# Cyruscxy/TinyPathTracer

Hardware: AMD Instinct MI355X
Metric: Mrays/s at 1920x1080x1024spp (box.gltf, 8 bounces); achieved GB/s vs peak (higher is better)
Workload: dtype f32

## Files before the change

### tinypathtracer_amd/csrc/common/device_api.hpp

```cpp
#pragma once

#include <hip/hip_runtime_api.h>
#include <stdint.h>

namespace tpt {

struct DevLight {
    int32_t type;
    float color[3];
    float intensity;
    float pos[3];
    float dir[3];
    float cos_outer;
    float inv_cos_cone_diff;
};

constexpr int kMaxLights = 16;
constexpr int kRngJumps = 16;
constexpr int kJumpWords = 160 * 5;

struct TraceArgs {
    const float4* inner;
    const float4* inner4;
    int32_t n4;
    int32_t lds_nodes;
    int32_t lds_nodes_offset;
    const float4* tri;
    const float4* shade;
    const float4* mtl;
    int32_t n_faces;
    int32_t n_materials;
    int32_t n_lights;
    int32_t stack_depth;
    const DevLight* lights;
    const uint32_t* env;
    int32_t env_w, env_h;
    int32_t is_b, is_bw, is_bh;
    const float* is_cond;
    const float* is_row;
    const float* is_marg;
    float is_total;
    const int32_t* is_guide_r;
    const int32_t* is_guide_c;
    int32_t is_kr, is_kc;
    int32_t env_is;
    float c2w[16];
    float origin[3];
    float sensor_w, sensor_h;
    float half_sw, half_sh;
    float inv_w, inv_h;
    int32_t width, height;
    int32_t band_rows, band_count, band_index, band_height;
    const int32_t* band_list;
    unsigned long long* band_cost;
    int32_t n_frames;
    int32_t max_depth;
    int32_t samples;
    int32_t flags;
    int32_t refill;
    int32_t leaf_kb;
    int32_t boxes_finite;
    int32_t any_emitter;
    int32_t emit_root;
    float4 emit_box[8];
    int32_t n_emit_box;
    const float4* sliver_groups;
    const float4* sliver_list;
    int32_t n_sliver_groups;
    float cull_eps;
    int32_t graze;
    int32_t pair;
    int32_t drained;
    int32_t quad;
    int32_t xcd_run;
    int32_t xcd_rot;
    int32_t lds_rec_offset;
    int32_t rec_lds_levels;
    int32_t stack_lds_slots;
    int32_t lds_stack_offset;
    int32_t lds_mtl_offset;
    int32_t mtl_in_lds;
    uint32_t* rng;
    float* accum;
    unsigned long long* counters;
    unsigned long long* debug_waves;
};

struct ResolveArgs {
    const float* accum;
    float* radiance;
    uint8_t* bgra;
    int32_t width, height;
    int32_t band_rows, band_count, band_index, band_height;
    const int32_t* band_list;
    int32_t spp;
};

hipError_t launch_rng_init(const uint32_t* jumps, uint64_t seed, int32_t width, int32_t band_rows,
                           int32_t band_count, int32_t band_index, const int32_t* band_list, int32_t band_height,
                           int32_t height, uint32_t* rng, hipStream_t s);
hipError_t launch_rng_init_linear(const uint32_t* jumps, uint64_t seed, uint64_t first, uint32_t n,
                                  uint32_t* states_aos, hipStream_t s);

struct BuildBuffers {
    int32_t n_faces, n_vertices, n_objects, n_materials;
    const uint32_t* indices;
    const float* vertices;
    const float* normals;
    const int2* lut;
    const float* vert_trans;
    const float* normal_trans;
    const float4* mtl;
    float* wverts;
    float* wnorms;
    unsigned long long* keys;
    unsigned long long* keys_sorted;
// ... 193 lines not shown
```

### tinypathtracer_amd/csrc/common/trace_variant.hpp

```cpp
#pragma once

#include <algorithm>
#include <cstddef>
#include <cstdint>
#include <type_traits>

#ifndef TPT_TRACE_WAVES
#define TPT_TRACE_WAVES 5
#endif
#ifndef TPT_TRACE_WAVES_IS
#define TPT_TRACE_WAVES_IS 4
#endif
#ifndef TPT_TRACE_WAVES_PAIR
#define TPT_TRACE_WAVES_PAIR 4
#endif
#ifndef TPT_TRACE_WAVES_DRAIN
#define TPT_TRACE_WAVES_DRAIN 4
#endif
#ifndef TPT_TRACE_WAVES_QUAD
#define TPT_TRACE_WAVES_QUAD 4
#endif

#ifdef TPT_WG_WAVES
#define TPT_WGW(n) TPT_WG_WAVES
#else
#define TPT_WGW(n) n
#endif
#define TPT_WGW_LANE TPT_WGW(1)
#define TPT_WGW_DRAIN TPT_WGW(1)
#define TPT_WGW_PAIR TPT_WGW(4)
#define TPT_WGW_IS TPT_WGW(4)
#define TPT_WGW_QUAD TPT_WGW(4)
#define TPT_WGW_REF TPT_WGW(4)
#ifndef TPT_MTL_LDS_MAX
#define TPT_MTL_LDS_MAX 2048
#endif

namespace tpt {

enum TraceFamily : int { TF_LANE, TF_DRAIN, TF_PAIR, TF_IS, TF_QUAD, TF_REF, TF_IS_PAIR, TF_REF_IS, kTraceFamilies };
constexpr int kTracePublicFamilies = 6;

struct TraceFamilyInfo {
    int wgw;
    int waves;
    int lds_waves;
    int lanes;
    int tile_w, tile_rows;
    bool env_is, ordered;
};
inline constexpr TraceFamilyInfo kTraceFamily[kTraceFamilies] = {
     {TPT_WGW_LANE, TPT_TRACE_WAVES, TPT_TRACE_WAVES, 1, 16, 16, false, true},
     {TPT_WGW_DRAIN, TPT_TRACE_WAVES_DRAIN, TPT_TRACE_WAVES, 1, 16, 16, false, true},
     {TPT_WGW_PAIR, TPT_TRACE_WAVES_PAIR, TPT_TRACE_WAVES_PAIR, 2, 16, 8, false, true},
     {TPT_WGW_IS, TPT_TRACE_WAVES_IS, TPT_TRACE_WAVES_IS, 1, 16, 16, true, true},
     {TPT_WGW_QUAD, TPT_TRACE_WAVES_QUAD, TPT_TRACE_WAVES_QUAD, 4, 8, 8, false, true},
     {TPT_WGW_REF, TPT_TRACE_WAVES, TPT_TRACE_WAVES, 1, 16, 16, false, false},
     {TPT_WGW_IS, TPT_TRACE_WAVES_IS, TPT_TRACE_WAVES_IS, 2, 16, 8, true, true},
     {TPT_WGW_REF, TPT_TRACE_WAVES_IS, TPT_TRACE_WAVES, 1, 16, 16, true, false},
};

struct TraceKey {
    TraceFamily family;
    bool deep;
    bool lights;
    bool mtl_lds;
    bool wide_ids;
    bool noemit;
};
constexpr int kTraceKeyBits = 8;
constexpr unsigned trace_key_pack(const TraceKey& k) {
    return (unsigned)k.family | k.deep << 3 | k.lights << 4 | k.mtl_lds << 5 | k.wide_ids << 6 | k.noemit << 7;
}
constexpr TraceKey trace_key_unpack(unsigned p) {
    return {(TraceFamily)(p & 7), (p >> 3 & 1) != 0, (p >> 4 & 1) != 0, (p >> 5 & 1) != 0, (p >> 6 & 1) != 0, (p >> 7 & 1) != 0};
}
constexpr bool trace_key_legal(const TraceKey& k) {
    const TraceFamilyInfo& f = kTraceFamily[k.family];
    if (!f.ordered && !(k.deep && k.lights && !k.mtl_lds && k.wide_ids)) return false;
    if (k.lights ? f.lanes == 4 : (f.lanes == 2 || f.env_is)) return false;
    return !k.noemit || f.lanes == 2;
}

template <TraceFamily F, int MAXD_, bool LIGHTS_, bool MTL_LDS_, typename StackT_, bool NOEMIT_>
struct TraceVariant {
    static_assert((MAXD_ == 8 || MAXD_ == 64) && (std::is_same_v<StackT_, uint16_t> || std::is_same_v<StackT_, int>));
    static constexpr TraceKey key{F, MAXD_ == 64, LIGHTS_, MTL_LDS_, sizeof(StackT_) == 4, NOEMIT_};
    static_assert(trace_key_legal(key), "no such k_trace variant (trace_key_legal)");
    static constexpr TraceFamilyInfo fam = kTraceFamily[F];
    static_assert(fam.wgw == 1 || fam.wgw == 2 || fam.wgw == 4, "waves per k_trace workgroup: 1, 2 or 4");
    static constexpr int MAXD = MAXD_, WGW = fam.wgw, WAVES = fam.waves;
    static constexpr bool ORDERED = fam.ordered, LIGHTS = LIGHTS_, MTL_LDS = MTL_LDS_, ENVIS = fam.env_is,
                          PAIR = fam.lanes == 2, DRAIN = F == TF_DRAIN, QUAD = fam.lanes == 4, NOEMIT = NOEMIT_;
    using StackT = StackT_;
};

constexpr uint32_t kNoProbe = 0x7fffu;
constexpr int rec_words(int n_lights, int n_materials) {
    return (n_lights > 0 || n_materials + 1 >= (int)kNoProbe) ? 5 : 2;
}
constexpr bool trace_small_ids(int n_faces) { return 2 * (size_t)n_faces - 1 <= 65535; }
constexpr bool trace_mtl_in_lds(int n_materials) { return (size_t)(n_materials + 1) * 32 <= (size_t)TPT_MTL_LDS_MAX; }
constexpr bool trace_five_words(bool ref_order, bool env_is, int n_lights, int n_materials) {
    return ref_order || env_is || rec_words(n_lights, n_materials) == 5;
}

struct TraceSelectIn {
    bool ref_order, env_is, pair, quad, drained;
    int n_lights, n_materials, n_faces, max_depth;
    bool any_emitter;
};
struct TraceSelection {
    TraceKey key;
    const char* error;
};
constexpr TraceSelection select_trace_variant(const TraceSelectIn& in) {
    if (in.ref_order) return {{in.env_is ? TF_REF_IS : TF_REF, true, true, false, true, false}, nullptr};
    const bool pair = in.pair && (in.env_is || in.n_lights > 0) && in.n_materials + 1 < (int)kNoProbe;
    TraceKey k{TF_LANE, in.max_depth > 8, trace_five_words(false, in.env_is, in.n_lights, in.n_materials),
               trace_mtl_in_lds(in.n_materials), !trace_small_ids(in.n_faces), pair && !in.any_emitter};
    if (in.env_is) k.family = pair ? TF_IS_PAIR : TF_IS;
    else if (in.quad) k.family = TF_QUAD;
    else if (pair) k.family = TF_PAIR;
    else if (in.drained) k.family = TF_DRAIN;
    return {k, trace_key_legal(k) ? nullptr : "four lanes per pixel need 2-word path records"};
}

struct TraceLds {
    size_t bytes;
    int mtl_offset, stack_offset, rec_offset;
    int stack_slots, rec_levels;
};
constexpr size_t kLdsSlack = 512;

inline TraceLds trace_lds_layout(const TraceKey& k, int wgw, int stack_depth, int max_depth, int n_materials,
                                 size_t max_slots = (size_t)-1, size_t max_levels = (size_t)-1) {
    const TraceFamilyInfo& f = kTraceFamily[k.family];
    size_t lds_budget = ((163840 / (size_t)f.lds_waves) & ~(size_t)255) * (size_t)wgw / 4;
    if (wgw < 4) lds_budget -= kLdsSlack * (size_t)wgw;
    const size_t row = 64 * (size_t)wgw;
    const size_t mtl_bytes = k.mtl_lds ? ((size_t)(n_materials + 1) * 2 * 16 + 127) / 128 * 128 : 0;
    const size_t budget = lds_budget - mtl_bytes;
    const size_t elem = k.wide_ids ? 4 : 2;
    const size_t slot = f.lanes == 4 ? row / 4 * elem : row * elem;
    const size_t level = (size_t)(k.lights ? 5 : 2) * (f.lanes == 2 ? row / 2 : row) * sizeof(float);
    size_t slots = std::min((size_t)stack_depth + 3, max_slots);
    const size_t want = std::min(std::min<size_t>((size_t)max_depth, (budget - 12 * slot) / level), max_levels);
    if (slots * slot + want * level > budget)
// ... 9 lines not shown
```

### tinypathtracer_amd/csrc/host/api_internal.hpp

```cpp
#pragma once

#include <hip/hip_runtime_api.h>

#include <algorithm>
#include <cstring>
#include <memory>
#include <string>
#include <thread>
#include <vector>

#include "../common/device_api.hpp"
#include "../common/ptrig.hpp"
#include "../common/tpt_math.hpp"
#include "launch_plan.hpp"
#include "tpt.h"
#include "tpt_internal.hpp"

namespace tpt {
namespace host __attribute__((visibility("hidden"))) {

tpt_status fail(tpt_status st, const std::string& msg);

#define HIP_OR_FAIL(expr)                                                                             \
    do {                                                                                              \
// ... 178 lines not shown
    int n4 = -1, need = 0, ne4 = -1, eneed = 0;
    tpt_status st = TPT_OK;
    std::string msg;
    tpt::WideWorkspace ws;
    std::thread th;
    ~HostTrees() { join(); }
    void join() {
        if (th.joinable()) th.join();
    }
    void reset_results() {
        n4 = -1;
        need = 0;
        ne4 = -1;
        eneed = 0;
        st = TPT_OK;
        msg.clear();
        prm.ws = &ws;
    }
    bool main_ok() const { return n4 > 0 && (size_t)n4 <= n - 1 && need <= 150; }
    int32_t base() const { return main_ok() ? n4 : lbvh_n4; }
    bool emit_ok() const { return ne4 > 0 && (size_t)(base() + ne4) <= n - 1 && eneed <= 150; }
};

std::vector<uint32_t>& host_jumps();
tpt_status finish_pending(tpt_scene* s, double* wait_ms = nullptr);
void fill_trace_args(tpt_scene* s, const tpt_env* env, const tpt_camera* cam, tpt::TraceArgs& a);
void fill_env_args(const tpt_env* env, tpt::TraceArgs& a);

}
}

using namespace tpt::host;

struct tpt_env {
    int device = 0;
    int w = 0, h = 0;
    DevBuf<uint32_t> texels;
    DevBuf<float> is_cond, is_row, is_marg;
    float is_total = 0.0f;
    int32_t is_b = 1, is_bw = 0, is_bh = 0;
    DevBuf<int32_t> is_guide_r, is_guide_c;
    int32_t is_kr = 1, is_kc = 1;
};

struct tpt_scene {
    int device = 0;
    hipStream_t stream = nullptr;
    hipEvent_t ev[4] = {nullptr, nullptr, nullptr, nullptr};
    int32_t n_faces = 0, n_vertices = 0, n_objects = 0, n_materials = 0, n_lights = 0;
    bool built = false;
    int32_t stack_depth = 0;
    int32_t boxes_finite = 0;
    int32_t any_emitter = 1;
    int32_t n4 = 0;
    int32_t wide_tree = 0;
    int32_t emit_root = -1;
    float emit_box[24] = {};
    int32_t n_emit_box = 0;
    int32_t slivers = 0;
    int32_t n_sliver_groups = 0;
    DevBuf<float4> sliver_groups, sliver_list;
    float cull_eps = 0.0f;
    uint32_t tree_depth = 0;
    int32_t build_threads = -1;
    DevBuf<uint8_t> sliver_flags;
    DevBuf<unsigned long long> coord_max;
    HostPinned<float> h_lbox;
    HostPinned<uint32_t> h_lemit;
    HostPinned<uint8_t> h_sliver;
    std::unique_ptr<HostTrees> trees;
    bool pending = false;
    uint32_t pending_need = 0;
    DevBuf<uint32_t> indices;
    DevBuf<float> vertices, normals, vert_trans, normal_trans;
    DevBuf<int2> lut;
    DevBuf<float4> mtl;
    DevBuf<tpt::DevLight> lights;
    DevBuf<uint32_t> jumps;
    std::vector<float> h_vert_trans;
    std::vector<int32_t> h_lut_begin;
    DevBuf<float> wverts, wnorms, leaf_box, node_box;
    DevBuf<unsigned long long> keys, keys_sorted, bfs_keys, bfs_keys_sorted;
    DevBuf<uint32_t> fids, fids_sorted, parent, flags, max_depth, bfs_ids, bfs_ids_sorted, bfs_newid, emit;
    DevBuf<int2> children;
    DevBuf<uint8_t> sort_tmp, nodes36;
    DevBuf<float4> inner, inner4, tri, shade;
    DevBuf<uint32_t> rng;
    DevBuf<float> accum, radiance_tmp;
    DevBuf<uint8_t> bgra_tmp;
    DevBuf<unsigned long long> counters, debug;
    size_t frame_pixels = 0;
    bool acc_valid = false;
    int acc_w = 0, acc_h = 0, acc_rows = 0, acc_count = 0, acc_index = 0;
    std::vector<int32_t> acc_list;
    uint64_t acc_spp = 0;
    DevBuf<int32_t> band_lists;
    std::vector<int32_t> band_lists_h;
    DevBuf<unsigned long long> band_cost;
    std::vector<unsigned long long> band_cost_h;
    int32_t n_cu = 0;
    uint64_t resident_lanes = 0;
    std::vector<uint64_t> acc_seeds;
    std::vector<hipStream_t> pipe;
    std::vector<hipEvent_t> lev;
    hipEvent_t pipe_ev[2 * tpt::kMaxPipe] = {};
    DevBuf<uint32_t> wf_state, wf_ctl;
// ... 84 lines not shown
```

### tinypathtracer_amd/csrc/host/api_render.cpp

```cpp
#include <chrono>
#include <cstdio>
#include <cstdlib>

#include "api_internal.hpp"

#ifndef TPT_XCD_ROT
#define TPT_XCD_ROT 1
#endif

void tpt::host::fill_env_args(const tpt_env* env, tpt::TraceArgs& a) {
    a.env = env ? env->texels.p : nullptr;
    a.env_w = env ? env->w : 0;
    a.env_h = env ? env->h : 0;
    a.is_b = env ? env->is_b : 1;
    a.is_bw = env ? env->is_bw : 0;
    a.is_bh = env ? env->is_bh : 0;
    a.is_cond = env ? env->is_cond.p : nullptr;
    a.is_row = env ? env->is_row.p : nullptr;
    a.is_marg = env ? env->is_marg.p : nullptr;
    a.is_total = env ? env->is_total : 0.0f;
    a.is_guide_r = env ? env->is_guide_r.p : nullptr;
    a.is_guide_c = env ? env->is_guide_c.p : nullptr;
    a.is_kr = env ? env->is_kr : 1;
    a.is_kc = env ? env->is_kc : 1;
}

void tpt::host::fill_trace_args(tpt_scene* s, const tpt_env* env, const tpt_camera* cam, tpt::TraceArgs& a) {
    a.inner = s->inner.p;
    a.inner4 = s->inner4.p;
    a.n4 = s->n4;
    a.tri = s->tri.p;
    a.shade = s->shade.p;
    a.mtl = s->mtl.p;
    a.n_faces = s->n_faces;
    a.n_materials = s->n_materials;
    a.n_lights = s->n_lights;
    a.lights = s->lights.p;
    a.stack_depth = s->stack_depth;
    a.boxes_finite = s->boxes_finite;
    a.any_emitter = s->any_emitter;
    a.emit_root = s->emit_root;
    a.n_emit_box = s->any_emitter ? s->n_emit_box : 0;
    for (int k = 0; k < a.n_emit_box; ++k) {
        const float* b = s->emit_box + 6 * k;
        a.emit_box[2 * k] = make_float4(b[0], b[1], b[2], 0.0f);
        a.emit_box[2 * k + 1] = make_float4(b[3], b[4], b[5], 0.0f);
    }
    a.sliver_groups = s->sliver_groups.p;
    a.sliver_list = s->sliver_list.p;
    a.n_sliver_groups = s->n_sliver_groups;
    a.cull_eps = s->cull_eps;
    a.graze = 1;
    fill_env_args(env, a);
    if (cam) set_camera(a, camera_consts(cam));
}

namespace {

tpt_status render_wavefront(tpt_scene* s, const tpt::TraceArgs& a, const tpt_params* p, int n_frames, int bh,
                            double& trace_ms, double& kernel_ms, int& launches) {
    hipStream_t st = s->stream;
    const bool ordered = !(p->flags & TPT_FLAG_REF_ORDER);
    const bool lights = tpt::trace_five_words(!ordered, a.env_is != 0, s->n_lights, s->n_materials);
    tpt::WfArgs w{};
    w.t = a;
    w.t.samples = p->spp;
    w.ordered = ordered ? 1 : 0;
    w.state_words = lights ? 32 : 16;
    w.rec_words = lights ? 5 : 2;
    const size_t gx = (size_t)(p->width + 15) / 16, gy = (size_t)((bh + 15) / 16) * (size_t)n_frames;
    const size_t claims = gx * gy * 256;
    if (bh <= 0) return TPT_OK;
    if (claims > (size_t)INT32_MAX / 2) return fail(TPT_ERR_INVALID_ARG, "wavefront: frame batch too large");
    if (p->wf_slots < 0 || p->wf_refill < 0 || p->wf_refill > 64)
        return fail(TPT_ERR_INVALID_ARG, "wavefront: wf_slots >= 0, wf_refill 0..64");
    size_t slots = p->wf_slots > 0 ? (size_t)p->wf_slots : claims;
    slots = std::min(slots, claims);
    slots = (slots + 255) / 256 * 256;
    w.n_claims = (int32_t)claims;
    w.n_slots = (int32_t)slots;
    HIP_OR_FAIL(s->wf_rec.alloc(slots * (size_t)p->max_depth * (size_t)w.rec_words));
    const size_t cap = ((slots / 256) + tpt::kWfShards - 1) / tpt::kWfShards * 256;
    const size_t qn = cap * tpt::kWfShards;
    HIP_OR_FAIL(s->wf_q0.alloc(2 * qn));
    HIP_OR_FAIL(s->wf_q1.alloc(2 * qn));
    HIP_OR_FAIL(s->wf_hit.alloc(qn));
    HIP_OR_FAIL(s->wf_state.alloc(2 * qn * (size_t)w.state_words));
    HIP_OR_FAIL(s->wf_ctl.alloc(tpt::kWfCtlWords));
    HIP_OR_FAIL(s->wf_count.alloc(2 * tpt::kWfShards));
    w.shard_cap = (int32_t)cap;
    for (auto& e : s->wf_ev)
        if (!e) HIP_OR_FAIL(hipEventCreateWithFlags(&e, hipEventDisableTiming));
    w.st0 = s->wf_state.p;
    w.st1 = s->wf_state.p + qn * (size_t)w.state_words;
// ... 378 lines not shown
```

### tinypathtracer_amd/csrc/host/api_scene.cpp

```cpp
#include <chrono>
#include <cmath>
#include <cstdio>
#include <cstdlib>
#include <new>
#include <system_error>

#include "../common/rng.hpp"
#include "../common/tri_rec.hpp"
#include "api_internal.hpp"

std::vector<uint32_t>& tpt::host::host_jumps() {
    static std::vector<uint32_t> j;
    if (j.empty()) {
        j.resize((size_t)tpt::kRngJumps * tpt::kJumpWords);
        tpt::xorwow_jump_matrices(tpt::kRngJumps, j.data());
    }
    return j;
}

namespace {

constexpr float kInfF = __builtin_huge_valf();

int env_is_block(int w, int h) {
// ... 424 lines not shown

    DeviceGuard g(device);
    tpt_scene_desc dh = *d_in;
    const tpt_scene_desc* d = &dh;
    std::vector<uint32_t> t_idx;
    std::vector<tpt_interval> t_lut;
    std::vector<float> t_vt, t_nt;
    std::vector<tpt_material> t_mtl;
    std::vector<tpt_light> t_lights;
    hipError_t herr = hipSuccess;
    dh.indices = host_view(d_in->indices, 3 * (size_t)d_in->n_faces, t_idx, &herr);
    dh.lut = host_view(d_in->lut, d_in->n_objects, t_lut, &herr);
    dh.vert_trans = host_view(d_in->vert_trans, 16 * (size_t)d_in->n_objects, t_vt, &herr);
    dh.normal_trans = host_view(d_in->normal_trans, 16 * (size_t)d_in->n_objects, t_nt, &herr);
    dh.materials = host_view(d_in->materials, d_in->n_materials, t_mtl, &herr);
    dh.lights = host_view(d_in->lights, d_in->n_lights, t_lights, &herr);
    if (herr != hipSuccess) return fail(TPT_ERR_HIP, std::string("scene desc readback: ") + hipGetErrorString(herr));
    int v_owner = -1, n_owner = -1;
    const bool verts_dev = is_device_ptr(d_in->vertices, &v_owner), norms_dev = is_device_ptr(d_in->normals, &n_owner);
    if ((v_owner >= 0 && v_owner != device) || (n_owner >= 0 && n_owner != device))
        return fail(TPT_ERR_INVALID_ARG, "device vertex/normal buffers must live on the scene's device");

    for (uint64_t i = 0; i < 3ull * d->n_faces; ++i)
        if (d->indices[i] >= d->n_vertices) return fail(TPT_ERR_INVALID_ARG, "vertex index out of range");
    if (d->lut[0].begin != 0) return fail(TPT_ERR_INVALID_ARG, "first object must begin at face 0");

    tpt_scene* s = new (std::nothrow) tpt_scene();
    if (!s) return fail(TPT_ERR_OOM, "host allocation failed");
    s->device = device;
    auto cleanup = [&](tpt_status st) {
        delete s;
        return st;
    };
    hipError_t e = hipStreamCreateWithFlags(&s->stream, hipStreamNonBlocking);
    for (int i = 0; e == hipSuccess && i < 4; ++i) e = hipEventCreate(&s->ev[i]);
    if (e != hipSuccess) return cleanup(fail(TPT_ERR_HIP, std::string("stream/event: ") + hipGetErrorString(e)));
    {
        hipDeviceProp_t prop{};
        e = hipGetDeviceProperties(&prop, device);
        if (e != hipSuccess) return cleanup(fail(TPT_ERR_HIP, std::string("device properties: ") + hipGetErrorString(e)));
        s->n_cu = prop.multiProcessorCount;
        s->resident_lanes = (uint64_t)std::max(s->n_cu, 1) * 4u * (uint64_t)tpt::trace_waves_per_simd() * 64u;
    }

    s->n_faces = (int32_t)d->n_faces;
    s->n_vertices = (int32_t)d->n_vertices;
    s->n_objects = (int32_t)d->n_objects;
    s->n_materials = (int32_t)d->n_materials;
    s->n_lights = (int32_t)d->n_lights;

    std::vector<int2> lut(d->n_objects);
    for (uint32_t i = 0; i < d->n_objects; ++i) lut[i] = make_int2(d->lut[i].begin, d->lut[i].mtl);
    std::vector<float4> mtl(2 * ((size_t)d->n_materials + 1));
    for (uint32_t i = 0; i <= d->n_materials; ++i) {
        tpt_material m = (i < d->n_materials && d->materials) ? d->materials[i] : tpt::default_material();
        mtl[2 * i] = make_float4(m.base_color[0], m.base_color[1], m.base_color[2], m.emission_factor);
        mtl[2 * i + 1] = make_float4(m.eta, m.metallic, 0.0f, 0.0f);
    }
    const bool union_layout = (d->flags & TPT_DESC_DELTALIGHT_LAYOUT) != 0;
    std::vector<tpt::DevLight> lights(d->n_lights);
    for (uint32_t i = 0; i < d->n_lights; ++i) {
        const tpt_light& L = d->lights[i];
        if (L.type < 0 || L.type > 2) return cleanup(fail(TPT_ERR_INVALID_ARG, "unknown delta light type"));
        tpt::DevLight& o = lights[i];
        o.type = L.type;
        std::memcpy(o.color, L.color, sizeof o.color);
        o.intensity = L.intensity;
        if (union_layout) {
            std::memset(o.pos, 0, sizeof o.pos);
            std::memset(o.dir, 0, sizeof o.dir);
            o.cos_outer = 0.0f;
            o.inv_cos_cone_diff = 0.0f;
            if (L.type == 1) {
                std::memcpy(o.dir, L.pos, sizeof o.dir);
            } else {
                std::memcpy(o.pos, L.pos, sizeof o.pos);
                if (L.type == 2) {
                    std::memcpy(o.dir, L.direction, sizeof o.dir);
                    o.cos_outer = L.cos_outer;
                    o.inv_cos_cone_diff = L.inv_cos_cone_diff;
                }
            }
        } else {
            std::memcpy(o.pos, L.pos, sizeof o.pos);
            std::memcpy(o.dir, L.direction, sizeof o.dir);
            o.cos_outer = L.cos_outer;
            o.inv_cos_cone_diff = L.inv_cos_cone_diff;
        }
    }
    const auto& jumps = host_jumps();
    hipStream_t st = s->stream;
    auto copy_in = [&](DevBuf<float>& dst, const float* src, size_t count, bool dev) {
        if (!dev) return dst.upload(src, count, st);
        hipError_t e2 = dst.alloc(count);
        if (e2 == hipSuccess) e2 = hipMemcpyAsync(dst.p, src, count * sizeof(float), hipMemcpyDeviceToDevice, st);
        return e2;
    };
    e = s->indices.upload(d->indices, 3 * (size_t)d->n_faces, st);
    if (e == hipSuccess) e = copy_in(s->vertices, d_in->vertices, 3 * (size_t)d->n_vertices, verts_dev);
    if (e == hipSuccess) e = copy_in(s->normals, d_in->normals, 3 * (size_t)d->n_vertices, norms_dev);
    if (e == hipSuccess) e = s->lut.upload(lut.data(), lut.size(), st);
    if (e == hipSuccess) e = s->vert_trans.upload(d->vert_trans, 16 * (size_t)d->n_objects, st);
    if (e == hipSuccess) e = s->normal_trans.upload(d->normal_trans, 16 * (size_t)d->n_objects, st);
    if (e == hipSuccess) e = s->mtl.upload(mtl.data(), mtl.size(), st);
    if (e == hipSuccess && !lights.empty()) e = s->lights.upload(lights.data(), lights.size(), st);
    if (e == hipSuccess) e = s->jumps.upload(jumps.data(), jumps.size(), st);
    if (e == hipSuccess) e = hipStreamSynchronize(st);
    if (e != hipSuccess)
// ... 109 lines not shown
```

### tinypathtracer_amd/csrc/kernels/trace.hip

```cpp
#include <array>
#include <map>
#include <mutex>
#include <type_traits>

#include "trace_dev.hpp"

namespace tpt {
#ifdef TPT_VERIFY_CULL
template <bool ORDERED>
__device__ __forceinline__ void trav_lane(Trav& r, const TraceArgs& a, LaneStack<int>& stk, uint32_t& c_ovf);
constexpr unsigned long long kVerifyCap = 4096;
__device__ __noinline__ void verify_ray(const TraceArgs& a, const Trav& r, int phase, const float4* mtl) {
    Trav q;
    trav_begin(q, r.o, r.d, TM_CLOSEST);
    LaneStack<int> vs;
    vs.lds = nullptr;
    vs.nlds = 0;
    uint32_t ovf = 0;
    trav_lane<false>(q, a, vs, ovf);
    bool bad;
    if (r.mode == TM_ANY) {
        bad = (q.fid >= 0) != (r.fid >= 0);
    } else if (r.mode == TM_CLOSEST && phase != 3) {
        bad = (q.fid != r.fid) || (__float_as_uint(q.t) != __float_as_uint(r.t)) ||
              (__float_as_uint(q.u) != __float_as_uint(r.u)) || (__float_as_uint(q.v) != __float_as_uint(r.v));
    } else {
        const float er = q.fid >= 0 ? mtl[2 * __float_as_int(a.shade[3 * q.fid].w)].w : 0.0f;
        const float eo = (r.fid >= 0 && r.mode != TM_OCCLUDED) ? mtl[2 * __float_as_int(a.shade[3 * r.fid].w)].w : 0.0f;
        bad = er != eo;
    }
    if (!bad) return;
    const unsigned long long k = atomicAdd(&a.counters[24], 1ull);
    if (k >= kVerifyCap || !a.debug_waves) return;
    unsigned long long* o = a.debug_waves + 16 * k;
    o[0] = (unsigned long long)r.mode;
    o[1] = (unsigned long long)phase;
    o[2] = (unsigned long long)(long long)r.fid;
    o[3] = (unsigned long long)(long long)q.fid;
    o[4] = __float_as_uint(r.t);
    o[5] = __float_as_uint(q.t);
    o[6] = __float_as_uint(r.o.x);
    o[7] = __float_as_uint(r.o.y);
    o[8] = __float_as_uint(r.o.z);
    o[9] = __float_as_uint(r.d.x);
    o[10] = __float_as_uint(r.d.y);
    o[11] = __float_as_uint(r.d.z);
    o[12] = (unsigned long long)(long long)r.hpos;
    o[13] = (unsigned long long)(long long)q.hpos;
    o[14] = __float_as_uint(r.u);
    o[15] = (unsigned long long)(r.fin ? 1u : 0u) | ((unsigned long long)__float_as_uint(r.lim) << 32);
}
#endif

template <class V>
__global__ __launch_bounds__(64 * V::WGW, V::WAVES) void k_trace(TraceArgs a) {
    constexpr int MAXD = V::MAXD;
    constexpr bool ORDERED = V::ORDERED, LIGHTS = V::LIGHTS, MTL_LDS = V::MTL_LDS, ENVIS = V::ENVIS, PAIR = V::PAIR,
                   DRAIN = V::DRAIN, QUAD = V::QUAD, NOEMIT = V::NOEMIT;
    using StackT = typename V::StackT;
    constexpr int WGW = V::WGW, NB = 4 / WGW, ROW = 64 * WGW;
    extern __shared__ __attribute__((aligned(16))) char lds[];
    const int tid = threadIdx.x, lane = tid & 63;
    const int nfr = a.n_frames > 0 ? a.n_frames : 1;
    int bx = (int)blockIdx.x / NB, part = (int)blockIdx.x % NB;
    const int by = (int)blockIdx.y;
    [[maybe_unused]] int tile_id = bx;
    if (a.xcd_run > 0) {
        const int b = (int)blockIdx.x, g = a.xcd_run, k = ((b & 7) + by + a.xcd_rot) & 7, m = (b >> 3) / NB;
        part = (b >> 3) % NB;
        tile_id = m * 8 + (b & 7);
        bx = ((m / g) * 8 + k) * g + m % g;
    }
    const int wave = part * WGW + (tid >> 6);
    const int frame = by % nfr;
    const bool side = PAIR && (lane & 1);
    const bool lead = !QUAD || (lane & 3) == 0;
    const int pl = PAIR ? (lane >> 1) : (QUAD ? (lane >> 2) : lane);
    const int x = QUAD ? bx * 8 + (wave & 1) * 4 + (pl & 3) : bx * 16 + (wave & 1) * 8 + (pl & 7);
    const int ly = PAIR   ? (by / nfr) * 8 + (wave >> 1) * 4 + (pl >> 3)
                   : QUAD ? (by / nfr) * 8 + (wave >> 1) * 4 + (pl >> 2)
                          : (by / nfr) * 16 + (wave >> 1) * 8 + (pl >> 3);
    const int y = band_row(ly, a.band_rows, a.band_count, a.band_index, a.band_list);
    const bool pixel = x < a.width && ly < a.band_height && y < a.height;
    const unsigned long long t_cost0 = a.band_cost ? wall_clock64() : 0ull;
    const bool active = pixel && !side;
    uint32_t c_trav = 0, c_inner = 0, c_wide = 0, c_leaf = 0, c_shade = 0, c_ovf = 0;
    uint32_t c_local = 0;
    const size_t npix = (size_t)a.width * (size_t)a.height;
    const size_t off = active ? (size_t)x + (size_t)y * (size_t)a.width : 0;
    uint32_t* const g_rng = a.rng + (size_t)frame * 6 * npix;
    float* const g_acc = a.accum + (size_t)frame * 3 * npix;
    const int nint = a.n_faces - 1;
    TPT_LDS char* slds = (TPT_LDS char*)lds;
    TPT_LDS LdsF4* smtl = (TPT_LDS LdsF4*)(slds + a.lds_mtl_offset);
    if constexpr (MTL_LDS) {
        for (int i = tid; i < 2 * (a.n_materials + 1); i += ROW) {
            const float4 m = a.mtl[i];
            smtl[i].x = m.x;
            smtl[i].y = m.y;
            smtl[i].z = m.z;
            smtl[i].w = m.w;
        }
    }
    TPT_LDS LdsF4* snodes = (TPT_LDS LdsF4*)(slds + a.lds_nodes_offset);
    for (int i = tid; i < 8 * a.lds_nodes; i += ROW) {
        const float4 m = a.inner4[i];
        snodes[i].x = m.x;
        snodes[i].y = m.y;
        snodes[i].z = m.z;
        snodes[i].w = m.w;
    }
// ... 9 lines not shown
        if constexpr (MTL_LDS) {
            return make_float4(smtl[i].x, smtl[i].y, smtl[i].z, smtl[i].w);
        } else {
            return a.mtl[i];
        }
    };
    LaneStack<StackT, QUAD, ROW> stk;
    stk.lds = (TPT_LDS StackT*)(slds + a.lds_stack_offset) + (QUAD ? (tid & ~3) : tid);
    stk.nlds = a.stack_lds_slots;
    PathRecords<MAXD, PAIR ? ROW / 2 : ROW> rec;
    rec.lds = (TPT_LDS float*)(slds + a.lds_rec_offset) + (PAIR ? (tid >> 6) * 32 + pl : tid);
    rec.nlds = a.rec_lds_levels;
    rec.words = LIGHTS ? 5 : 2;

    uint32_t st[6];
    V3 total = v3(0.0f, 0.0f, 0.0f);
    if (active) {
#pragma unroll
        for (int i = 0; i < 6; ++i) st[i] = g_rng[i * npix + off];
        total = v3(g_acc[off], g_acc[npix + off], g_acc[2 * npix + off]);
    }
    int remaining = a.samples;
    int phase = PH_CAMERA;
    int depth = 0, li = 0;
    uint32_t mk = 0;
    bool env_pending = false;
    V3 env_k = v3(0.0f, 0.0f, 0.0f);
    float env_x1 = 0.0f, env_x2 = 0.0f;
    V3 env_nf = v3(0.0f, 0.0f, 0.0f);
    V3 rd = v3(0.0f, 0.0f, 0.0f), nd = rd, nrm = rd, direct = rd;
    Trav r;
    trav_begin(r, rd, v3(1.0f, 1.0f, 1.0f), TM_CLOSEST);
    int ts = active ? TS_DONE : ((PAIR && side && pixel) ? TS_IDLE : TS_DEAD);
#ifdef TPT_VERIFY_CULL
    bool vpend = false;
#endif
    bool sl_pend = false;
    Surf gsurf = no_surface();
    bool graze_next = false;
    float4 pq0 = make_float4(0.0f, 0.0f, 0.0f, 0.0f), pq1 = pq0, pq2 = pq0;
    const int refill = a.refill;
    bool delegated = false, post = false, ready = false;
    bool post_env = false;
    int pend = -1, jlevel = 0;
    auto put_level = [&](uint32_t pm, V3 dl) {
        if constexpr (PAIR) {
            rec.template put_dst<true>(depth, mk, pm, dl);
            if (!delegated) {
                rec.put(depth, 2, direct.x);
                rec.put(depth, 3, direct.y);
                rec.put(depth, 4, direct.z);
            }
        } else {
            rec.put_dst(depth, mk, pm, dl);
        }
    };

#ifdef TPT_PROFILE_PHASES
    const unsigned long long t_wave0 = wall_clock64();
    unsigned long long p_done = 0, p_trav = 0, p_steps = 0, t_iter0 = 0, t_loop0 = 0, p_outer = 0;
    unsigned long long p_lt = 0, p_lw = 0, p_lx = 0, p_lp = 0;
    unsigned int p_sec[8] = {0, 0, 0, 0, 0, 0, 0, 0};
    unsigned long long t_sec = 0;
    bool p_lead = false;
#endif
#ifdef TPT_PROFILE_PHASES
#define TPT_SEC_BEGIN()                                                       \
    {                                                                         \
        __builtin_amdgcn_s_waitcnt(0);                                        \
        t_sec = wall_clock64();                                               \
        p_lead = __builtin_amdgcn_readfirstlane(lane) == lane;                \
    }
#define TPT_SEC(k)                                                            \
    {                                                                         \
        __builtin_amdgcn_s_waitcnt(0);                                        \
        const unsigned long long t_ = wall_clock64();                         \
        if (p_lead) p_sec[k] += (unsigned int)(t_ - t_sec);                   \
        t_sec = t_;                                                           \
    }
#else
#define TPT_SEC_BEGIN()
#define TPT_SEC(k)
#endif
    for (;;) {
#ifdef TPT_PROFILE_PHASES
        {
            const unsigned long long now = wall_clock64();
            if (t_loop0) p_trav += now - t_loop0;
            t_iter0 = now;
        }
#endif
        if (ORDERED && a.n_sliver_groups > 0) {
            if (ts == TS_DONE && sl_pend) {
                sl_pend = false;
                sliver_pass(r, a, c_leaf);
            }
        }
        if (ORDERED && !NOEMIT && ts == TS_DONE && phase == PH_PROBE && r.fin && r.fid >= 0 && r.mode == TM_EMIT &&
            a.graze && grazing(Surf{a.shade[3 * r.fid + 1].w, a.shade[3 * r.fid + 2].w}, r.d)) {
            trav_begin(r, r.o, r.d, r.mode, a.boxes_finite != 0, a.emit_root, a.cull_eps, true);
            ts = TS_TRAV;
            sl_pend = false;
        }
        if (ORDERED && !NOEMIT && ts == TS_DONE && phase == PH_PROBE && r.mode == TM_EMIT && r.fid >= 0) {
            r.mode = TM_OCCL;
            r.node = 0;
            r.sp = 0;
            r.pend = -1;
            ts = TS_TRAV;
            sl_pend = true;
        }
#ifdef TPT_VERIFY_CULL
        if (ts == TS_DONE && vpend) {
            vpend = false;
            if (!(phase == PH_EXT && r.fin && r.fid >= 0 && a.graze &&
                  grazing(Surf{a.shade[3 * r.fid + 1].w, a.shade[3 * r.fid + 2].w}, r.d)))
                verify_ray(a, r, phase, a.mtl);
        }
#endif
#ifdef TPT_PROFILE_PHASES
        if (__ballot(ts == TS_DONE) != 0ull) p_lp += (unsigned long long)__popcll(__ballot(ts == TS_DONE));
#endif
        const bool in_pass = ts == TS_DONE;
        bool finish = false;
        bool redo = false;
        bool shadow = false;
        bool tg = false;
        V3 L = v3(0.0f, 0.0f, 0.0f), td = rd;
        if (in_pass) {
            TPT_SEC_BEGIN()
            bool lights_next = false, after = false;
            if (!LIGHTS) rd = r.d;
            Surf gpass = gsurf;
            if (phase == PH_EXT) {
                if (r.fid < 0) {
                    if (a.env) L = env_lookup<ENVIS>(a.env, a.env_w, a.env_h, rd);
                    finish = true;
                } else {
                    const float4* sh = a.shade + 3 * r.fid;
                    const float4 s0 = sh[0], s1 = sh[1], s2 = sh[2];
                    redo = ORDERED && r.fin && a.graze && grazing(Surf{s1.w, s2.w}, rd);
                    if (!redo) {
                        ++c_shade;
                        const float w = 1.0f - r.u - r.v;
                        nrm = normalize(((w * v3(s0.x, s0.y, s0.z)) + (r.u * v3(s1.x, s1.y, s1.z))) +
                                        (r.v * v3(s2.x, s2.y, s2.z)));
                        gpass = a.graze ? Surf{s1.w, s2.w} : no_surface();
                        if constexpr (LIGHTS) gsurf = gpass;
                        r.o = r.o + (r.t * rd);
                        const int mtl = __float_as_int(s0.w);
                        const float4 m1 = MT(2 * mtl + 1);
                        float af;
                        const float prob = new_direction(rd, nrm, m1.x, m1.y, st, nd, af);
                        graze_next = grazing(gpass, nd);
                        rec.put(depth, 0, af);
                        mk = (uint32_t)mtl | (p_kind(prob) << 30);
                        direct = v3(0.0f, 0.0f, 0.0f);
                        li = 0;
                        delegated = false;
                        env_pending = ENVIS && !(m1.x > 0.0f) && !(m1.y > 0.0f);
                        lights_next = true;
                    }
                }
            } else if (LIGHTS && phase == PH_SHADOW) {
                if (r.fid < 0) {
                    V3 ldir, lrad;
                    light_sample(a.lights, li, r.o, ldir, lrad);
                    const float4 m0 = MT(2 * (mk & 0x3fffffffu));
                    direct = direct + (v3(m0.x, m0.y, m0.z) * lrad);
                }
                ++li;
                lights_next = true;
            } else if (ENVIS && phase == PH_ENVSHADOW) {
                if (r.fid < 0) direct = direct + env_k;
                lights_next = true;
            } else if (!NOEMIT && phase == PH_PROBE) {
                V3 dl = LIGHTS ? direct : v3(0.0f, 0.0f, 0.0f);
                uint32_t pm = kNoProbe;
                if (r.fid >= 0 && r.mode != TM_OCCLUDED) {
                    pm = (uint32_t)__float_as_int(a.shade[3 * r.fid].w);
                    const float e = MT(2 * pm).w;
                    if (!PAIR) dl = (v3(1.0f, 1.0f, 1.0f) * v3(e, e, e)) + dl;
                }
                put_level(pm, dl);
                after = true;
            } else if (PAIR && phase == PH_WAIT) {
                L = direct;
                finish = true;
            }
            TPT_SEC(1)
            td = rd;
            tg = redo;
            if (PAIR && lights_next && !side && li == 0 && pend < 0 && (a.n_lights > 0 || (ENVIS && env_pending))) {
                post = true;
                jlevel = depth;
                pend = depth;
                delegated = true;
                li = a.n_lights;
                if (ENVIS && env_pending) {
                    env_pending = false;
                    env_x1 = xorwow_uniform(st);
                    env_x2 = xorwow_uniform(st);
                    env_nf = (dot(rd, nrm) > 0.0f ? -1.0f : 1.0f) * nrm;
                    post_env = true;
                }
            }
            if (PAIR && lights_next && side && li >= a.n_lights && !(ENVIS && env_pending)) {
                ready = true;
                ts = TS_IDLE;
                lights_next = false;
            }
            if (lights_next) {
                const float4 m1 = MT(2 * (mk & 0x3fffffffu) + 1);
                if (LIGHTS && li < a.n_lights) {
                    V3 lrad;
                    light_sample(a.lights, li, r.o, td, lrad);
                    tg = grazing(gsurf, td);
                    phase = PH_SHADOW;
                    shadow = true;
                } else {
                    bool env_ray = false;
                    if (ENVIS && env_pending) {
                        env_pending = false;
                        V3 nf = env_nf;
                        float x1 = env_x1, x2 = env_x2;
                        if (!(PAIR && side)) {
                            nf = (dot(rd, nrm) > 0.0f ? -1.0f : 1.0f) * nrm;
                            x1 = xorwow_uniform(st);
                            x2 = xorwow_uniform(st);
                        }
                        if (env_is_sample(a, nf, x1, x2, td, env_k)) {
                            phase = PH_ENVSHADOW;
                            shadow = true;
                            env_ray = true;
                            tg = grazing(gsurf, td);
                        }
                    }
                    if (env_ray) {
                    } else if (PAIR && side) {
                        ready = true;
                        ts = TS_IDLE;
                    } else if (!(m1.x >= 1.0f || m1.y > 0.0f)) {
                        float af2;
                        new_direction(rd, nrm, m1.x, m1.y, st, td, af2);
                        if ((ORDERED && (NOEMIT || !a.any_emitter)) ||
                            (ORDERED && probe_misses_emitters(a, r.o, td))) {
                            ++c_trav;
                            ++c_local;
                            put_level(kNoProbe, direct);
                            after = true;
                        } else {
                            tg = grazing(gpass, td);
                            phase = PH_PROBE;
                        }
                    } else {
                        put_level(kNoProbe, direct);
                        after = true;
                    }
                }
            }
            TPT_SEC(2)
            if (after) {
                const float e = MT(2 * (mk & 0x3fffffffu)).w;
                if (e > 0.0f) {
                    L = e * v3(1.0f, 1.0f, 1.0f);
                    finish = true;
                } else {
                    rd = nd;
                    td = rd;
                    tg = graze_next;
                    ++depth;
                    if (depth == a.max_depth) finish = true;
                    else phase = PH_EXT;
                }
            }
            TPT_SEC(3)
        }
        bool woke = false;
        if constexpr (PAIR && ENVIS) {
            const int jready = __shfl_xor((int)ready, 1, 64);
            const float dx = __shfl_xor(direct.x, 1, 64), dy = __shfl_xor(direct.y, 1, 64),
                        dz = __shfl_xor(direct.z, 1, 64);
            const int rl = __shfl_xor(jlevel, 1, 64);
            if (!side && jready) {
                rec.put(rl, 2, dx);
                rec.put(rl, 3, dy);
                rec.put(rl, 4, dz);
                pend = -1;
                if (!in_pass && phase == PH_WAIT) {
                    woke = true;
                    ts = TS_DONE;
                    L = direct;
                    finish = true;
                    td = rd;
                }
            }
            ready = false;
        }
        if (in_pass || woke) {
            if (PAIR && finish && pend >= 0) {
                direct = L;
                phase = PH_WAIT;
                ts = TS_IDLE;
                finish = false;
            }
            bool unwound = false;
            if constexpr (DRAIN && !LIGHTS && MAXD == 8) {
                static_assert(!PAIR && !LIGHTS, "DRAIN unwind: one-lane 2-word records");
                if (finish && rec.nlds >= 8) {
                    unwound = true;
                    float af[8];
                    uint32_t w1[8];
#pragma unroll
                    for (int k = 0; k < 8; ++k) {
                        af[k] = rec.template lds_at<2>(k, 0);
                        w1[k] = k < depth ? __float_as_uint(rec.template lds_at<2>(k, 1)) : (kNoProbe << 15);
                    }
                    float4 mb[8];
                    float ee[8];
#pragma unroll
                    for (int k = 0; k < 8; ++k) {
                        mb[k] = MT(2 * (w1[k] & 0x7fffu));
                        const uint32_t pm = (w1[k] >> 15) & 0x7fffu;
                        ee[k] = MT(2 * (pm == kNoProbe ? 0u : pm)).w;
                    }
#pragma unroll
                    for (int k = 7; k >= 0; --k) {
                        if (k < depth) {
                            const V3 att = af[k] * v3(mb[k].x, mb[k].y, mb[k].z);
                            const uint32_t kind = w1[k] >> 30;
                            const float prob = kind == 0u ? af[k] : (kind == 1u ? -0.0f : 0.0f);
                            const float ivp = 1.0f / prob;
                            const uint32_t pm = (w1[k] >> 15) & 0x7fffu;
                            const float e = pm == kNoProbe ? 0.0f : ee[k];
                            const V3 dst = pm == kNoProbe ? v3(0.0f, 0.0f, 0.0f)
                                                          : (v3(1.0f, 1.0f, 1.0f) * v3(e, e, e)) + v3(0.0f, 0.0f, 0.0f);
                            L = ivp * ((dst + L) * att);
                        }
                    }
                    total = total + L;
                    phase = PH_CAMERA;
                }
            }
            if (finish && !unwound) {
                for (int k = depth - 1; k >= 0; --k) {
                    const float af = rec.get(k, 0);
                    const uint32_t w1 = __float_as_uint(rec.get(k, 1));
                    const bool packed = rec.words == 2;
                    const float4 mb = MT(2 * (w1 & ((packed || PAIR) ? 0x7fffu : 0x3fffffffu)));
                    const V3 att = af * v3(mb.x, mb.y, mb.z);
                    const uint32_t kind = w1 >> 30;
                    const float prob = kind == 0u ? af : (kind == 1u ? -0.0f : 0.0f);
                    const float ivp = 1.0f / prob;
                    V3 dst;
                    if (packed) {
                        const uint32_t pm = (w1 >> 15) & 0x7fffu;
                        const float e = pm == kNoProbe ? 0.0f : MT(2 * pm).w;
                        dst = pm == kNoProbe ? v3(0.0f, 0.0f, 0.0f)
                                             : (v3(1.0f, 1.0f, 1.0f) * v3(e, e, e)) + v3(0.0f, 0.0f, 0.0f);
                    } else if (PAIR) {
                        const uint32_t pm = (w1 >> 15) & 0x7fffu;
                        const V3 dd = v3(rec.get(k, 2), rec.get(k, 3), rec.get(k, 4));
                        const float e = pm == kNoProbe ? 0.0f : MT(2 * pm).w;
                        dst = pm == kNoProbe ? dd : (v3(1.0f, 1.0f, 1.0f) * v3(e, e, e)) + dd;
                    } else {
                        dst = v3(rec.get(k, 2), rec.get(k, 3), rec.get(k, 4));
                    }
                    L = ivp * ((dst + L) * att);
                }
                total = total + L;
                phase = PH_CAMERA;
            }
            TPT_SEC(4)
            V3 to = r.o;
            if (phase == PH_CAMERA) {
                if (remaining == 0) {
                    ts = TS_DEAD;
                } else {
                    --remaining;
                    const float ju = xorwow_uniform(st);
                    const float jv = xorwow_uniform(st);
                    float lx = ju * 1.0f, lyf = jv * 1.0f;
                    lx = lx + (float)x;
                    lyf = lyf + (float)y;
                    lx = lx * a.inv_w;
                    lyf = lyf * a.inv_h;
                    lx = lx * a.sensor_w;
                    lyf = lyf * a.sensor_h;
                    float r4[4];
                    mat4_vec4(a.c2w, lx - a.half_sw, lyf - a.half_sh, 0.0f - 1.0f, 0.0f, r4);
                    rd = normalize(v3(r4[0], r4[1], r4[2]));
                    td = rd;
                    to = v3(a.origin[0], a.origin[1], a.origin[2]);
                    tg = false;
                    depth = 0;
                    phase = PH_EXT;
                }
            }
            TPT_SEC(5)
            if (ts != TS_DEAD && ts != TS_IDLE) {
                if (!redo) ++c_trav;
                trav_begin(r, to, td, shadow ? TM_ANY : ((ORDERED && phase == PH_PROBE) ? TM_EMIT : TM_CLOSEST),
                           a.boxes_finite != 0, a.emit_root, a.cull_eps, tg);
                ts = TS_TRAV;
                sl_pend = true;
#ifdef TPT_VERIFY_CULL
                vpend = true;
#endif
            }
            TPT_SEC(6)
        }
        if constexpr (PAIR) {
            const int jpost = __shfl_xor((int)post, 1, 64);
            const float jx = __shfl_xor(r.o.x, 1, 64), jy = __shfl_xor(r.o.y, 1, 64), jz = __shfl_xor(r.o.z, 1, 64);
            const int jmk = __shfl_xor((int)mk, 1, 64), jl = __shfl_xor(jlevel, 1, 64);
            const Surf jgs = Surf{__shfl_xor(gsurf.x, 1, 64), __shfl_xor(gsurf.y, 1, 64)};
            bool jenv = false;
            if constexpr (ENVIS) {
                jenv = __shfl_xor((int)post_env, 1, 64) != 0;
                const float e1 = __shfl_xor(env_x1, 1, 64), e2 = __shfl_xor(env_x2, 1, 64);
                const float n0 = __shfl_xor(env_nf.x, 1, 64), n1 = __shfl_xor(env_nf.y, 1, 64),
                            n2 = __shfl_xor(env_nf.z, 1, 64);
                if (side && jpost) {
                    env_pending = jenv;
                    env_x1 = e1;
                    env_x2 = e2;
                    env_nf = v3(n0, n1, n2);
                }
            }
            if (side && jpost) {
                mk = (uint32_t)jmk;
                jlevel = jl;
                gsurf = jgs;
                li = 0;
                direct = v3(0.0f, 0.0f, 0.0f);
                V3 ldir, lrad;
                const V3 jo = v3(jx, jy, jz);
                bool go = true;
                if (a.n_lights > 0) {
                    light_sample(a.lights, 0, jo, ldir, lrad);
                    phase = PH_SHADOW;
                } else if (ENVIS && env_pending) {
                    env_pending = false;
                    go = env_is_sample(a, env_nf, env_x1, env_x2, ldir, env_k);
                    phase = PH_ENVSHADOW;
                } else {
                    go = false;
                }
// ... 85 lines not shown
                        const TriQ tq = tri_load(a.tri, r.pend);
                        pq0 = tq.q0;
                        pq1 = tq.q1;
                        pq2 = tq.q2;
                    }
                }
                has = r.pend >= 0;
                inner_ready = r.node >= 0 && r.node < nint;
                blocked = has && !inner_ready;
            }
            const unsigned long long hb = __ballot(has);
            if (hb != 0ull) {
                const bool go = __popcll(__ballot(blocked)) >= a.leaf_kb || __popcll(hb) >= TPT_LEAF_KP ||
                                __ballot(inner_ready) == 0ull;
                if (go && has) {
                    ++c_leaf;
                    const bool stop = DRAIN ? leaf_test_q<ORDERED>(r, pq0, pq1, pq2, r.pend, a.cull_eps)
                                            : leaf_test<ORDERED>(r, a.tri, r.pend, a.cull_eps);
                    if (stop) {
                        r.node = -1;
                        r.sp = 0;
                    }
                    r.pend = -1;
                }
            }
            if (ts == TS_TRAV && r.node < 0 && r.pend < 0) ts = TS_DONE;
        }
    }
    if (active && lead) {
#pragma unroll
        for (int i = 0; i < 6; ++i) g_rng[i * npix + off] = st[i];
        g_acc[off] = total.x;
        g_acc[npix + off] = total.y;
        g_acc[2 * npix + off] = total.z;
    }
    if (!lead) {
        c_trav = c_inner = c_wide = c_leaf = c_shade = c_ovf = c_local = 0;
    }
    const unsigned long long s_wide = wave_sum(c_wide), s_local = wave_sum(c_local);
    const unsigned long long s_trav = wave_sum(c_trav), s_inner = wave_sum(c_inner), s_leaf = wave_sum(c_leaf),
                             s_shade = wave_sum(c_shade), s_ovf = wave_sum(c_ovf);
#ifdef TPT_PROFILE_PHASES
    unsigned long long m_trav = c_trav;
#pragma unroll
    for (int off = 32; off > 0; off >>= 1) {
        const unsigned long long o2 = __shfl_xor(m_trav, off, 64);
        m_trav = o2 > m_trav ? o2 : m_trav;
    }
#endif
#ifdef TPT_PROFILE_PHASES
    unsigned long long s_sec[7];
#pragma unroll
    for (int k = 0; k < 7; ++k) s_sec[k] = wave_sum(p_sec[k]);
    if (lane == 0) {
#pragma unroll
        for (int k = 0; k < 7; ++k) atomicAdd(&a.counters[16 + k], s_sec[k]);
    }
#endif
    if (lane == 0) {
        atomicAdd(&a.counters[0], s_trav);
        atomicAdd(&a.counters[1], s_inner);
        atomicAdd(&a.counters[2], s_leaf);
        atomicAdd(&a.counters[3], s_shade);
        if (s_ovf) atomicAdd(&a.counters[4], s_ovf);
        atomicAdd(&a.counters[5], s_wide);
        atomicAdd(&a.counters[9], s_local);
        if (a.band_cost && ly < a.band_height)
            atomicAdd(&a.band_cost[band_of(ly / a.band_rows, a.band_count, a.band_index, a.band_list)],
                      wall_clock64() - t_cost0);
#ifdef TPT_PROFILE_PHASES
        atomicAdd(&a.counters[6], p_done);
        atomicAdd(&a.counters[7], p_trav);
        atomicAdd(&a.counters[8], p_steps);
        atomicAdd(&a.counters[12], p_outer);
        atomicAdd(&a.counters[25], p_lt);
        atomicAdd(&a.counters[26], p_lw);
        atomicAdd(&a.counters[27], p_lx);
        atomicAdd(&a.counters[28], p_lp);
        const unsigned long long life = wall_clock64() - t_wave0;
        atomicMax(&a.counters[13], life);
        atomicAdd(&a.counters[14], life);
        atomicAdd(&a.counters[15], 1ull);
        if (a.debug_waves) {
            const unsigned long long wid =
                ((unsigned long long)blockIdx.y * (gridDim.x / NB) + tile_id) * 4 + wave;
            unsigned long long* o = a.debug_waves + 8 * wid;
            o[0] = t_wave0;
            o[1] = life;
            o[2] = p_steps;
            o[3] = p_outer;
            o[4] = s_trav;
            o[5] = s_wide;
            o[6] = m_trav;
            o[7] = p_done;
        }
#endif
    }
}

__global__ void k_resolve(ResolveArgs a) {
    const int x = blockIdx.x * blockDim.x + threadIdx.x;
    const int ly = blockIdx.y;
    if (x >= a.width || ly >= a.band_height) return;
    const int y = band_row(ly, a.band_rows, a.band_count, a.band_index, a.band_list);
    if (y >= a.height) return;
    const size_t npix = (size_t)a.width * (size_t)a.height;
    const size_t off = (size_t)x + (size_t)y * (size_t)a.width;
    const float inv = 1.0f / (float)a.spp;
    const float r = (0.0f + a.accum[off]) * inv;
    const float g = (0.0f + a.accum[npix + off]) * inv;
    const float b = (0.0f + a.accum[2 * npix + off]) * inv;
    if (a.radiance) {
        a.radiance[3 * off] = r;
        a.radiance[3 * off + 1] = g;
        a.radiance[3 * off + 2] = b;
    }
    if (a.bgra) {
        uint8_t* px = a.bgra + 4 * ((size_t)(a.height - y - 1) * (size_t)a.width + (size_t)x);
        px[0] = to_uchar(b);
        px[1] = to_uchar(g);
        px[2] = to_uchar(r);
    }
}

constexpr int kRaysLdsSlots = 48;

__global__ __launch_bounds__(256) void k_trace_rays(TraceArgs a, uint32_t n, const float* __restrict__ o,
                                                    const float* __restrict__ d, const int32_t* __restrict__ ofid,
                                                    int mode, int32_t* hit, float* t, float* uv) {
    extern __shared__ __attribute__((aligned(16))) char lds[];
    const uint32_t i = blockIdx.x * 256 + threadIdx.x;
// ... 366 lines not shown
```

Baseline: 16080.

## Prune zero-radiance path unwinding by tracking the deepest contributing bounce

For the ordered, no-lights variants, packs into the material word the depth of the last bounce that can still contribute (a probe or a non-trivial throughput factor). When a path finishes with zero radiance, unwinding is truncated to that depth. If no lane in the wave needs any unwinding, the whole DRAIN unwind block is skipped. This removes per-bounce record reads and multiplies for dead paths, at the cost of narrowing the material-id field to 15 bits and adding host checks on material colours to enable it.

```diff
diff --git a/tinypathtracer_amd/csrc/common/device_api.hpp b/tinypathtracer_amd/csrc/common/device_api.hpp
--- a/tinypathtracer_amd/csrc/common/device_api.hpp
+++ b/tinypathtracer_amd/csrc/common/device_api.hpp
@@ -62,6 +62,7 @@
     int32_t boxes_finite;
     int32_t any_emitter;
     int32_t emit_root;
+    int32_t unwind_prune;
     float4 emit_box[8];
     int32_t n_emit_box;
     const float4* sliver_groups;
diff --git a/tinypathtracer_amd/csrc/common/trace_variant.hpp b/tinypathtracer_amd/csrc/common/trace_variant.hpp
--- a/tinypathtracer_amd/csrc/common/trace_variant.hpp
+++ b/tinypathtracer_amd/csrc/common/trace_variant.hpp
@@ -3,6 +3,7 @@
 #include <algorithm>
 #include <cstddef>
 #include <cstdint>
+#include <cstring>
 #include <type_traits>
 
 #ifndef TPT_TRACE_WAVES
@@ -92,8 +93,16 @@
     static constexpr int MAXD = MAXD_, WGW = fam.wgw, WAVES = fam.waves;
     static constexpr bool ORDERED = fam.ordered, LIGHTS = LIGHTS_, MTL_LDS = MTL_LDS_, ENVIS = fam.env_is,
                           PAIR = fam.lanes == 2, DRAIN = F == TF_DRAIN, QUAD = fam.lanes == 4, NOEMIT = NOEMIT_;
+    static constexpr bool PRUNE = !LIGHTS_ && ORDERED && !PAIR && !ENVIS;
     using StackT = StackT_;
 };
+
+constexpr float kPruneAfMin = 0x1p-100f, kPruneAfMax = 0x1p100f, kPruneColorCap = 0x1p27f;
+inline bool prune_color_ok(float c) {
+    uint32_t b;
+    std::memcpy(&b, &c, sizeof b);
+    return b <= 0x4d000000u;
+}
 
 constexpr uint32_t kNoProbe = 0x7fffu;
 constexpr int rec_words(int n_lights, int n_materials) {
diff --git a/tinypathtracer_amd/csrc/host/api_internal.hpp b/tinypathtracer_amd/csrc/host/api_internal.hpp
--- a/tinypathtracer_amd/csrc/host/api_internal.hpp
+++ b/tinypathtracer_amd/csrc/host/api_internal.hpp
@@ -254,6 +254,7 @@
     int32_t stack_depth = 0;
     int32_t boxes_finite = 0;
     int32_t any_emitter = 1;
+    int32_t unwind_prune = 0;
     int32_t n4 = 0;
     int32_t wide_tree = 0;
     int32_t emit_root = -1;
diff --git a/tinypathtracer_amd/csrc/host/api_render.cpp b/tinypathtracer_amd/csrc/host/api_render.cpp
--- a/tinypathtracer_amd/csrc/host/api_render.cpp
+++ b/tinypathtracer_amd/csrc/host/api_render.cpp
@@ -40,6 +40,10 @@
     a.boxes_finite = s->boxes_finite;
     a.any_emitter = s->any_emitter;
     a.emit_root = s->emit_root;
+    a.unwind_prune = s->unwind_prune;
+#ifdef TPT_PROFILE_PHASES
+    if (std::getenv("TPT_DEBUG_NO_PRUNE")) a.unwind_prune = 0;
+#endif
     a.n_emit_box = s->any_emitter ? s->n_emit_box : 0;
     for (int k = 0; k < a.n_emit_box; ++k) {
         const float* b = s->emit_box + 6 * k;
diff --git a/tinypathtracer_amd/csrc/host/api_scene.cpp b/tinypathtracer_amd/csrc/host/api_scene.cpp
--- a/tinypathtracer_amd/csrc/host/api_scene.cpp
+++ b/tinypathtracer_amd/csrc/host/api_scene.cpp
@@ -500,8 +500,11 @@
     std::vector<int2> lut(d->n_objects);
     for (uint32_t i = 0; i < d->n_objects; ++i) lut[i] = make_int2(d->lut[i].begin, d->lut[i].mtl);
     std::vector<float4> mtl(2 * ((size_t)d->n_materials + 1));
+    s->unwind_prune = 1;
     for (uint32_t i = 0; i <= d->n_materials; ++i) {
         tpt_material m = (i < d->n_materials && d->materials) ? d->materials[i] : tpt::default_material();
+        for (int c = 0; c < 3; ++c)
+            if (!tpt::prune_color_ok(m.base_color[c])) s->unwind_prune = 0;
         mtl[2 * i] = make_float4(m.base_color[0], m.base_color[1], m.base_color[2], m.emission_factor);
         mtl[2 * i + 1] = make_float4(m.eta, m.metallic, 0.0f, 0.0f);
     }
diff --git a/tinypathtracer_amd/csrc/kernels/trace.hip b/tinypathtracer_amd/csrc/kernels/trace.hip
--- a/tinypathtracer_amd/csrc/kernels/trace.hip
+++ b/tinypathtracer_amd/csrc/kernels/trace.hip
@@ -56,7 +56,8 @@
 __global__ __launch_bounds__(64 * V::WGW, V::WAVES) void k_trace(TraceArgs a) {
     constexpr int MAXD = V::MAXD;
     constexpr bool ORDERED = V::ORDERED, LIGHTS = V::LIGHTS, MTL_LDS = V::MTL_LDS, ENVIS = V::ENVIS, PAIR = V::PAIR,
-                   DRAIN = V::DRAIN, QUAD = V::QUAD, NOEMIT = V::NOEMIT;
+                   DRAIN = V::DRAIN, QUAD = V::QUAD, NOEMIT = V::NOEMIT, PRUNE = V::PRUNE;
+    constexpr uint32_t kZTop = PRUNE ? 0x7fu << 15 : 0u, kMkId = PRUNE ? 0x7fffu : 0x3fffffffu;
     using StackT = typename V::StackT;
     constexpr int WGW = V::WGW, NB = 4 / WGW, ROW = 64 * WGW;
     extern __shared__ __attribute__((aligned(16))) char lds[];
@@ -172,7 +173,10 @@
                 rec.put(depth, 4, direct.z);
             }
         } else {
-            rec.put_dst(depth, mk, pm, dl);
+            if constexpr (PRUNE) {
+                if (pm != kNoProbe) mk = (mk & ~kZTop) | (uint32_t)(depth + 1) << 15;
+            }
+            rec.put_dst(depth, mk & ~kZTop, pm, dl);
         }
     };
 
@@ -180,6 +184,7 @@
     const unsigned long long t_wave0 = wall_clock64();
     unsigned long long p_done = 0, p_trav = 0, p_steps = 0, t_iter0 = 0, t_loop0 = 0, p_outer = 0;
     unsigned long long p_lt = 0, p_lw = 0, p_lx = 0, p_lp = 0;
+    uint32_t p_uw_iter = 0, p_uw_lane = 0, p_uw_pass = 0;
     unsigned int p_sec[8] = {0, 0, 0, 0, 0, 0, 0, 0};
     unsigned long long t_sec = 0;
     bool p_lead = false;
@@ -274,7 +279,13 @@
                         const float prob = new_direction(rd, nrm, m1.x, m1.y, st, nd, af);
                         graze_next = grazing(gpass, nd);
                         rec.put(depth, 0, af);
-                        mk = (uint32_t)mtl | (p_kind(prob) << 30);
+                        if constexpr (PRUNE) {
+                            const uint32_t kind = p_kind(prob);
+                            const bool clean = kind == 0u && af >= kPruneAfMin && af <= kPruneAfMax;
+                            mk = (uint32_t)mtl | (kind << 30) | (clean ? (mk & kZTop) : (uint32_t)(depth + 1) << 15);
+                        } else {
+                            mk = (uint32_t)mtl | (p_kind(prob) << 30);
+                        }
                         direct = v3(0.0f, 0.0f, 0.0f);
                         li = 0;
                         delegated = false;
@@ -331,7 +342,7 @@
                 lights_next = false;
             }
             if (lights_next) {
-                const float4 m1 = MT(2 * (mk & 0x3fffffffu) + 1);
+                const float4 m1 = MT(2 * (mk & kMkId) + 1);
                 if (LIGHTS && li < a.n_lights) {
                     V3 lrad;
                     light_sample(a.lights, li, r.o, td, lrad);
@@ -381,7 +392,7 @@
             }
             TPT_SEC(2)
             if (after) {
-                const float e = MT(2 * (mk & 0x3fffffffu)).w;
+                const float e = MT(2 * (mk & kMkId)).w;
                 if (e > 0.0f) {
                     L = e * v3(1.0f, 1.0f, 1.0f);
                     finish = true;
@@ -425,9 +436,29 @@
                 finish = false;
             }
             bool unwound = false;
+            if constexpr (PRUNE) {
+                const uint32_t lbits = __float_as_uint(L.x) | __float_as_uint(L.y) | __float_as_uint(L.z);
+                if (finish && a.unwind_prune && lbits == 0u) depth = min(depth, (int)((mk & kZTop) >> 15));
+            }
+#ifdef TPT_PROFILE_PHASES
+            {
+                uint32_t mt = 0;
+                while (__ballot(finish && depth > (int)mt) != 0ull) ++mt;
+                if (__builtin_amdgcn_readfirstlane(lane) == lane) {
+                    p_uw_iter += mt;
+                    p_uw_pass += mt > 0u ? 1u : 0u;
+                }
+                p_uw_lane += finish ? (uint32_t)depth : 0u;
+            }
+#endif
             if constexpr (DRAIN && !LIGHTS && MAXD == 8) {
                 static_assert(!PAIR && !LIGHTS, "DRAIN unwind: one-lane 2-word records");
-                if (finish && rec.nlds >= 8) {
+                if (finish && rec.nlds >= 8 && __ballot(finish && depth > 0) == 0ull) {
+                    unwound = true;
+                    total = total + L;
+                    phase = PH_CAMERA;
+                }
+                if (finish && !unwound && rec.nlds >= 8) {
                     unwound = true;
                     float af[8];
                     uint32_t w1[8];
@@ -514,6 +545,7 @@
                     to = v3(a.origin[0], a.origin[1], a.origin[2]);
                     tg = false;
                     depth = 0;
+                    if constexpr (PRUNE) mk = 0;
                     phase = PH_EXT;
                 }
             }
@@ -705,6 +737,7 @@
     unsigned long long s_sec[7];
 #pragma unroll
     for (int k = 0; k < 7; ++k) s_sec[k] = wave_sum(p_sec[k]);
+    const unsigned long long s_uw[3] = {wave_sum(p_uw_iter), wave_sum(QUAD && !lead ? 0u : p_uw_lane), wave_sum(p_uw_pass)};
     if (lane == 0) {
 #pragma unroll
         for (int k = 0; k < 7; ++k) atomicAdd(&a.counters[16 + k], s_sec[k]);
@@ -730,6 +763,9 @@
         atomicAdd(&a.counters[26], p_lw);
         atomicAdd(&a.counters[27], p_lx);
         atomicAdd(&a.counters[28], p_lp);
+        atomicAdd(&a.counters[29], s_uw[0]);
+        atomicAdd(&a.counters[30], s_uw[1]);
+        atomicAdd(&a.counters[31], s_uw[2]);
         const unsigned long long life = wall_clock64() - t_wave0;
         atomicMax(&a.counters[13], life);
         atomicAdd(&a.counters[14], life);
```

Measured after the change: 16640 (median of 6 runs). +3.5%, better.
